# tingiskhan/pyfilter

Hardware: AMD Instinct MI355X
Metric: particle-steps/sec (batch x particles x T), 1M-particle APF (higher is better)
Workload: dtype f32; 1 GPU; apf_lgo_1m: APF + lgo proposal, systematic resampling, N=1048576 particles x B=1 filters per GPU, T=250, state dim 1; parallelism=single GPU

## Files before the change

### pyfilter_amd/csrc/pf_fused.hpp

```cpp
#pragma once

namespace pf {

#define PF_STEP_B blockIdx.x
#define PF_STEP_K blockIdx.y

#ifdef PF_DEVTOOLS
#define PF_CUT(a, n) ((a).debug_cut == (n))
#define PF_STAMP(a, slot)                                                                       \
    do {                                                                                        \
        if ((a).debug_cut < 0 && !(a).finalize_only && PF_STEP_K == (unsigned)(-(a).debug_cut - 1) &&  \
            PF_STEP_B == 0 && threadIdx.x == 0)                                                 \
            (a).dbg[slot] = (unsigned long long)clock64();                                      \
    } while (0)
#else
#define PF_CUT(a, n) false
#ifdef PF_ISA_MARKS
#define PF_STAMP(a, slot) asm volatile("; PF_MARK " #slot)
#else
#define PF_STAMP(a, slot) do { } while (0)
#endif
#endif

template <typename T> struct FusedArgs {
    ModelDesc md;
    const T* params;
    int filter, proposal, resampler;
    Geom g;
    double thr_abs;
    double logN;
    T rcN;
    uint64_t seed;
    const uint64_t* seed_dev;
    T* x[2];
    T* logw[2];
    int32_t* anc;
    const int32_t* anc_prev;
    T* cdf;
    T* pos;
    const T* y;
    int y_rows;
    const T* z_tape;
    const T* u_tape;
    const T* user_loc;
    const T* user_scale;
    int user_scale_percol;
    T user_dt;
    T* means;
    T* vars;
    T* ll_steps;
    T* ll_total;
    double* part;
    int64_t part_stride;
    ColStat* stat;
    int32_t* poison;
    T* cpack;
    double* piv0;
    double* ctab;
    int64_t ctab_stride;
    int t0;
    int step;
    int obs;
    int obs_next;
    const uint8_t* obs_dev;
    __device__ __forceinline__ bool y_informative() const {
        const T* yr = y + (int64_t)step * md.obs_dim;
        bool any = false;
        for (int o = 0; o < md.obs_dim; ++o) any = any || !(yr[o] != yr[o]);
        return any;
    }
    __device__ __forceinline__ bool is_obs() const { return obs >= 0 ? obs != 0 : (obs == -1 ? obs_dev[step] != 0 : y_informative()); }
    __device__ __forceinline__ bool is_obs_next() const { return obs_next >= 0 ? obs_next != 0 : obs_dev[step + 1] != 0; }
    int finalize_only;
    int book_inline;
    unsigned kmap;
    __device__ __forceinline__ int tile_of_row(unsigned y) const {
        return (int)(((y & (kmap & 0xffu)) << ((kmap >> 8) & 0xffu)) + (y >> ((kmap >> 16) & 0xffu)));
    }
    unsigned long long* dbg;
    __device__ __forceinline__ const double* part_r() const { return part + (int64_t)(step & 1) * part_stride; }
    __device__ __forceinline__ double* part_w(int state) const { return part + (int64_t)(state & 1) * part_stride; }
    __device__ __forceinline__ const double* ctab_r(int b) const {
        return ctab + (int64_t)(step & 1) * ctab_stride + (int64_t)b * g.tiles * g.rounds_per_tile * PF_NWAVES * 2;
    }
    __device__ __forceinline__ double* ctab_w(int state, int b) const {
        return ctab + (int64_t)(state & 1) * ctab_stride + (int64_t)b * g.tiles * g.rounds_per_tile * PF_NWAVES * 2;
    }
    template <int D> __device__ __forceinline__ T pivot(int q, int b, int d) const {
        return (q - 2 >= t0) ? means[((int64_t)(q - 2) * g.B + b) * D + d] : (T)piv0[(int64_t)b * PF_MAXD + d];
    }
    int debug_cut;
};

template <typename T, int D>
__device__ __forceinline__ void load_col_params(const FusedArgs<T>& a, int b, int step, bool with_y, ColParams<T, D>& cp,
                                                int late = 0) {
    const int O = a.md.obs_dim;
    const int NP = 4 * D + O * D + 2 * O;
    cp.load(a.params + (int64_t)b * NP + late, O,
            with_y ? a.y + ((int64_t)step * a.y_rows + (a.y_rows == 1 ? 0 : b)) * O + late : nullptr);
}

template <typename T, int D, bool WQ = true> struct PartialAcc {
    T m1, m2;
    T s1, s2, q1;
    T mx[D], mxx[D];
    double es;
    bool poison;
    __device__ __forceinline__ void init() {
        m1 = m2 = -Lim<T>::inf();
        s1 = s2 = q1 = T(0);
        es = 0.0;
#pragma unroll
        for (int d = 0; d < D; ++d) mx[d] = mxx[d] = T(0);
        poison = false;
    }
    template <int VEC>
    __device__ __forceinline__ void push_round(const T (&lw)[VEC], const T (&x)[D][VEC], bool pre_on, const T (&pre)[VEC],
                                               const T (&piv)[D], T (&e_out)[VEC]) {
        T m = lw[0];
#pragma unroll
        for (int j = 1; j < VEC; ++j) m = (lw[j] > m) ? lw[j] : m;
        if (m > m1) {
            const T rs = (m1 == -Lim<T>::inf()) ? T(0) : pf_exp_w(m1 - m);
            s1 *= rs;
            if constexpr (WQ) q1 *= rs * rs;
#pragma unroll
            for (int d = 0; d < D; ++d) {
                mx[d] *= rs;
                mxx[d] *= rs;
            }
            m1 = m;
        }
#pragma unroll
        for (int j = 0; j < VEC; ++j) {
            T e = (lw[j] == -Lim<T>::inf()) ? T(0) : pf_exp_w(lw[j] - m1);
            if (lw[j] != lw[j]) e = lw[j];
            e_out[j] = e;
            s1 += e;
            if constexpr (WQ) q1 += e * e;
#pragma unroll
            for (int d = 0; d < D; ++d) {
                const T xd = x[d][j] - piv[d];
                mx[d] += e * xd;
                mxx[d] += e * xd * xd;
            }
        }
        if (pre_on) {
            T rw[VEC];
#pragma unroll
            for (int j = 0; j < VEC; ++j) {
                if (is_nan_or_posinf(pre[j])) poison = true;
                rw[j] = sanitize_logw(pre[j] + lw[j]);
            }
            T mm = rw[0];
#pragma unroll
            for (int j = 1; j < VEC; ++j) mm = (rw[j] > mm) ? rw[j] : mm;
            if (mm > m2) {
                s2 *= (m2 == -Lim<T>::inf()) ? T(0) : pf_exp_w(m2 - mm);
                m2 = mm;
            }
#pragma unroll
            for (int j = 0; j < VEC; ++j) {
                const T e = (rw[j] == -Lim<T>::inf()) ? T(0) : pf_exp_w(rw[j] - m2);
                e_out[j] = e;
                s2 += e;
            }
        }
    }
    template <bool WITH_ES>
    __device__ __forceinline__ void finish(double* part, int b, int k, int B, int tiles, bool pre_on, double* red, T* redm,
                                           int32_t* poison_slot, T& M1_out, T& M2_out, T& F1_out, T& F2_out) {
        const int lane = threadIdx.x & 63, wid = threadIdx.x >> 6;
        const T w1 = wave_max<T>(m1), w2 = wave_max<T>(m2);
        if (lane == 0) {
            redm[wid] = w1;
            redm[PF_NWAVES + wid] = w2;
        }
        __syncthreads();
        T M1 = redm[0], M2 = redm[PF_NWAVES];
#pragma unroll
        for (int w = 1; w < PF_NWAVES; ++w) {
            M1 = (redm[w] > M1) ? redm[w] : M1;
            M2 = (redm[PF_NWAVES + w] > M2) ? redm[PF_NWAVES + w] : M2;
        }
        M1_out = M1;
        M2_out = M2;
        const T f1 = (m1 == -Lim<T>::inf()) ? T(0) : pf_exp_w(m1 - M1);
        const T f2 = (!pre_on || m2 == -Lim<T>::inf()) ? T(0) : pf_exp_w(m2 - M2);
        F1_out = f1;
        F2_out = f2;
        constexpr int NS = 3 + 2 * D;
        T sums[NS];
        sums[0] = s1 * f1;
        sums[1] = WQ ? q1 * f1 * f1 : T(0);
        sums[2] = pre_on ? s2 * f2 : T(0);
#pragma unroll
        for (int d = 0; d < D; ++d) {
            sums[3 + d] = mx[d] * f1;
            sums[3 + D + d] = mxx[d] * f1;
        }
#pragma unroll
        for (int q = 0; q < NS; ++q) {
            const T ws = (WQ || q != 1) ? wave_sum(sums[q]) : T(0);
            if (lane == 0) red[q * PF_NWAVES + wid] = (double)ws;
        }
        if constexpr (WITH_ES) {
            const double ws = wave_sum(es);
            if (lane == 0) red[NS * PF_NWAVES + wid] = ws;
        }
        if (poison) atomicOr(poison_slot, 1);
        __syncthreads();
        if (threadIdx.x < NS + 1) {
            const int q = threadIdx.x;
            double r = 0.0;
            if (q < NS || WITH_ES) {
                r = red[q * PF_NWAVES];
#pragma unroll
                for (int w = 1; w < PF_NWAVES; ++w) r += red[q * PF_NWAVES + w];
            }
            const int row = q == 0 ? PQ_S1 : q == 1 ? PQ_Q1 : q == 2 ? PQ_S2 : q == NS ? PQ_E : PQ_MX + (q - 3);
            const int64_t stride = (int64_t)B * tiles;
            const int64_t o = (int64_t)b * tiles + k;
            part[row * stride + o] = r;
            if (q == 0) {
                part[PQ_M1 * stride + o] = (double)M1;
                part[PQ_M2 * stride + o] = pre_on ? (double)M2 : -__builtin_huge_val();
            }
        }
    }
};

#define PF_LDS_CHUNKS PF_WAVE
template <typename T>
__device__ __forceinline__ T cdf_from_local(T L, double Pk, double fk, double Pnext, bool tile_last, bool col_last) {
    double c = Pk + fk * (double)L;
    if (c > Pnext) c = Pnext;
    T r = (T)c;
    if (tile_last) r = col_last ? T(1) : (T)Pnext;
    return r;
}
template <typename T>
__device__ __forceinline__ T cdf_from_local(T L, double C, double gq, double Pk, double fk, double Pnext, bool tile_last,
                                            bool col_last) {
    double c = Pk + fk * (C + gq * (double)L);
    if (c > Pnext) c = Pnext;
    T r = (T)c;
    if (tile_last) r = col_last ? T(1) : (T)Pnext;
    return r;
}
template <typename T> struct CdfView {
    const T* L;
    const double* ptab;
    const double* ftab;
    const double* ct;
    int chunk_elems;
    int N;
    int tile_elems;
    int tiles;
    __device__ __forceinline__ int lower_bound(int from, T p, int kt_lo) const {
        if (from >= N) return N;
        int lo = kt_lo, hi = tiles - 1;
        while (lo < hi) {
            const int mid = (lo + hi) >> 1;
            if ((T)ptab[mid + 1] < p) lo = mid + 1; else hi = mid;
        }
        for (int kt = lo; kt < tiles; ++kt) {
            const int first = kt * tile_elems;
            const int end = first + tile_elems < N ? first + tile_elems : N;
            int a = from > first ? from : first, b = end;
            if (a >= b) continue;
            const double Pk = ptab[kt], fk = ftab[kt], Pn = ptab[kt + 1];
            while (a < b) {
                const int mid = (a + b) >> 1;
                T cv;
                if (ct) {
                    const double* cg = ct + 2 * (mid / chunk_elems);
                    cv = cdf_from_local<T>(L[mid], cg[0], cg[1], Pk, fk, Pn, mid == end - 1, mid == N - 1);
                } else {
                    cv = cdf_from_local<T>(L[mid], Pk, fk, Pn, mid == end - 1, mid == N - 1);
                }
                if (cv < p) a = mid + 1; else b = mid;
            }
            if (a < end) return a;
        }
        return N;
    }
};

template <typename T, int VEC, bool WT = false>
__device__ __forceinline__ void chunk_scan_round(const T (&rw)[VEC], bool on, T* __restrict__ l_base, int l_elem, int chunk,
                                                 double* lds_rec, double* raw) {
    T* const l_dst = l_base + l_elem;
    const int lane = threadIdx.x & 63;
    T mt = rw[0];
// ... 71 lines not shown
    const Geom& g = a.g;
    const int b = blockIdx.y, k = blockIdx.x;
    const int slot = a.step & 1;
    const bool pre_on = a.is_obs() && a.filter == PF_FILTER_APF;
    const bool user = a.md.hid_kind == PF_HID_USER_AFFINE;
    ColParams<T, D> cp;
    load_col_params<T, D>(a, b, a.step, pre_on, cp);
    ColConsts<T, D> cc;
    cc.prepare(a.md, cp);
    if (user && a.user_scale_percol) cc.prepare_user(a.md, cp, a.user_scale[b]);

    const T* lw_col = a.logw[slot] + (int64_t)b * g.N;
    const T* x_base = a.x[slot];
    T piv[D];
#pragma unroll
    for (int d = 0; d < D; ++d) piv[d] = x_base[((int64_t)d * g.B + b) * g.N];
    if (k == 0 && threadIdx.x == 0) {
#pragma unroll
        for (int d = 0; d < D; ++d) a.piv0[(int64_t)b * PF_MAXD + d] = (double)piv[d];
    }
    if constexpr (D == 1) {
        if (k == 0 && threadIdx.x == PF_BLOCK - 1 && a.md.obs_kind == PF_OBS_LINEAR && a.md.hid_kind != PF_HID_VERHULST_EM) {
            ColParams<T, 1> cq;
            ColConsts<T, 1> cd;
            load_col_params<T, 1>(a, b, a.step, false, cq);
            cd.prepare(a.md, cq);
            write_col_pack<T>(a.md, cq, cd, a.cpack + (int64_t)b * PK_N);
        }
    }
    PartialAcc<T, D> acc;
    acc.init();
    __shared__ double reds[PF_NWAVES];
    __shared__ double crec[2 * PF_LDS_CHUNKS];
    const bool use_lds = g.rounds_per_tile * PF_NWAVES <= PF_LDS_CHUNKS;
    double* const ct_tile = a.ctab_w(a.step, b) + 2 * (int64_t)k * g.rounds_per_tile * PF_NWAVES;
    T* const l_col = ((a.step & 1) ? a.pos : a.cdf) + (int64_t)b * g.N;
    const int64_t base = (int64_t)k * g.tile_elems;
    int rk = 0;
    for (int r = 0; r < g.rounds_per_tile; ++r) {
        const int64_t r0 = base + (int64_t)r * g.round_elems;
        if (r0 >= g.N) break;
        ++rk;
        const int64_t i0 = r0 + threadIdx.x * VEC;
        const bool on = i0 < g.N;
        T rw[VEC];
#pragma unroll
        for (int j = 0; j < VEC; ++j) rw[j] = -Lim<T>::inf();
        if (on) {
            T lw[VEC], xv[D][VEC];
            if (VEC == 1) lw[0] = lw_col[i0]; else load_vec<T, VEC>(lw_col + i0, lw);
#pragma unroll
            for (int d = 0; d < D; ++d) {
                const T* xc = x_base + ((int64_t)d * g.B + b) * g.N + i0;
                if (VEC == 1) xv[d][0] = xc[0]; else load_vec<T, VEC>(xc, xv[d]);
            }
            T pre[VEC];
#pragma unroll
            for (int j = 0; j < VEC; ++j) {
                T xj[D];
#pragma unroll
                for (int d = 0; d < D; ++d) xj[d] = xv[d][j];
                UserMS<T, D> um = UserMS<T, D>::none();
                if (user && pre_on) {
                    um.gather(a.user_loc, a.user_scale, (int64_t)b * g.N, (int64_t)g.B * g.N, i0 + j, a.user_scale_percol != 0, b, g.B);
                    um.euler(xj, a.user_dt);
                }
                pre[j] = pre_on ? pre_weight<T, D>(a.md, a.proposal, cp, cc, xj, false, um) : T(0);
                if (pre_on && is_nan_or_posinf(pre[j])) acc.poison = true;
                rw[j] = pre_on ? sanitize_logw(pre[j] + lw[j]) : lw[j];
            }
            T e_unused[VEC];
            acc.template push_round<VEC>(lw, xv, false, pre, piv, e_unused);
            if (a.resampler == PF_RESAMPLE_MULTINOMIAL) {
                T ev[VEC];
                draw_exponentials<T, VEC>(a.seed + (a.seed_dev ? *a.seed_dev : 0ull), PF_STREAM_MULTINOMIAL, (uint32_t)a.step,
                                          (uint64_t)((int64_t)b * g.N + i0), ev);
#pragma unroll
                for (int j = 0; j < VEC; ++j) acc.es += (double)ev[j];
            }
        }
        chunk_scan_round<T, VEC>(rw, on, l_col + r0, threadIdx.x * VEC, r * PF_NWAVES + (threadIdx.x >> 6), use_lds ? crec : nullptr, ct_tile);
    }
    T M1, M2, F1, F2;
    acc.template finish<true>(a.part_w(a.step), b, k, g.B, g.tiles, false, red, redm, &a.poison[(a.step & 3) * g.B + b], M1, M2, F1, F2);
    double Mc, Sc;
    finalize_chunk_table<T>(ct_tile, use_lds ? crec : nullptr, rk * PF_NWAVES, reds, redm, Mc, Sc);
    if (threadIdx.x == 0) {
        const int64_t stride = (int64_t)g.B * g.tiles, o = (int64_t)b * g.tiles + k;
        if (pre_on) {
            a.part_w(a.step)[PQ_M2 * stride + o] = Mc;
            a.part_w(a.step)[PQ_S2 * stride + o] = Sc;
        } else {
            a.part_w(a.step)[PQ_S1 * stride + o] = Sc;
        }
    }
    if (g.rounds_per_tile == 1) {
        __syncthreads();
        const int64_t i0 = base + threadIdx.x * VEC;
        if (i0 < g.N) {
            const double* cg = ct_tile + 2 * (threadIdx.x >> 6);
            const double C = cg[0], gq = cg[1];
            T v[VEC];
            if (VEC == 1) v[0] = l_col[i0]; else load_vec<T, VEC>(l_col + i0, v);
#pragma unroll
            for (int j = 0; j < VEC; ++j) v[j] = (T)(C + gq * (double)v[j]);
            if (VEC == 1) l_col[i0] = v[0]; else store_vec<T, VEC>(l_col + i0, v);
        }
    }
}

#define PF_COMBINE_ITERS (PF_MAX_TILES / PF_BLOCK)
template <typename T> __device__ __forceinline__ double pf_rcp_tot(double tot) {
    if constexpr (sizeof(T) == 4) {
        double r = __builtin_amdgcn_rcp(tot);
        r = __builtin_fma(__builtin_fma(-tot, r, 1.0), r, r);
        r = __builtin_fma(__builtin_fma(-tot, r, 1.0), r, r);
        return r;
    }
    return 1.0 / tot;
}
#define PF_PROBE_STEP 8
struct ColSums {
    double M, S, Q;
};
template <bool WITH_Q, int NX> struct ColPartials {
    double m[PF_COMBINE_ITERS], s[PF_COMBINE_ITERS], q[PF_COMBINE_ITERS];
    double x[NX ? NX : 1][PF_COMBINE_ITERS];
};
template <bool WITH_Q, int NX = 0>
__device__ __forceinline__ void load_col_partials(const double* part, int64_t stride, int64_t cb, int tiles, int slot_m,
                                                  int slot_s, int slot_x, ColPartials<WITH_Q, NX>& r) {
    const int IT = (tiles + PF_BLOCK - 1) / PF_BLOCK;
    if constexpr (PF_COMBINE_ITERS == 4 && NX == 0) {
        if (IT == 4 && (tiles & 3) == 0) {
            const int t0 = threadIdx.x * 4;
            if (t0 < tiles) {
                double a2[2], b2[2];
                const double* pm = part + slot_m * stride + cb + t0;
                load_vec<double, 2>(pm, a2); load_vec<double, 2>(pm + 2, b2);
                r.m[0] = a2[0]; r.m[1] = a2[1]; r.m[2] = b2[0]; r.m[3] = b2[1];
                const double* ps = part + slot_s * stride + cb + t0;
                load_vec<double, 2>(ps, a2); load_vec<double, 2>(ps + 2, b2);
                r.s[0] = a2[0]; r.s[1] = a2[1]; r.s[2] = b2[0]; r.s[3] = b2[1];
                if constexpr (WITH_Q) {
                    const double* pq = part + PQ_Q1 * stride + cb + t0;
                    load_vec<double, 2>(pq, a2); load_vec<double, 2>(pq + 2, b2);
                    r.q[0] = a2[0]; r.q[1] = a2[1]; r.q[2] = b2[0]; r.q[3] = b2[1];
                } else {
                    r.q[0] = r.q[1] = r.q[2] = r.q[3] = 0.0;
                }
            } else {
#pragma unroll
                for (int q = 0; q < 4; ++q) { r.m[q] = -__builtin_huge_val(); r.s[q] = 0.0; r.q[q] = 0.0; }
            }
            return;
        }
    }
#pragma unroll
    for (int q = 0; q < PF_COMBINE_ITERS; ++q) {
        const int t = threadIdx.x * IT + q;
        const bool on = q < IT && t < tiles;
        r.m[q] = on ? part[slot_m * stride + cb + t] : -__builtin_huge_val();
        r.s[q] = on ? part[slot_s * stride + cb + t] : 0.0;
        r.q[q] = (WITH_Q && on) ? part[PQ_Q1 * stride + cb + t] : 0.0;
#pragma unroll
        for (int i = 0; i < NX; ++i) r.x[i][q] = on ? part[(slot_x + i) * stride + cb + t] : 0.0;
    }
// ... 598 lines not shown
                    const double Ca = cga[0], ga = cga[1], Cb = cgb[0], gb = cgb[1];
#pragma unroll
                    for (int j = 0; j < VEC; ++j) {
                        const bool tl = (j == VEC - 1) && (wja + j == la);
                        m0[j] = wina ? cdf_from_local<T>(m0[j], Ca, ga, tPa, tFa, tNa, tl, tl && (wja + j == N - 1)) : Lim<T>::inf();
                    }
#pragma unroll
                    for (int j = 0; j < V1; ++j)
                        m1[j] = winb ? cdf_from_local<T>(m1[j], Cb, gb, tPb, tFb, tNb, wjb + j == lb, wjb + j == N - 1) : Lim<T>::inf();
                } else {
#pragma unroll
                    for (int j = 0; j < VEC; ++j) {
                        const bool tl = (j == VEC - 1) && (wja + j == la);
                        m0[j] = wina ? cdf_from_local<T>(m0[j], tPa, tFa, tNa, tl, tl && (wja + j == N - 1)) : Lim<T>::inf();
                    }
#pragma unroll
                    for (int j = 0; j < V1; ++j)
                        m1[j] = winb ? cdf_from_local<T>(m1[j], tPb, tFb, tNb, wjb + j == lb, wjb + j == N - 1) : Lim<T>::inf();
                }
            };
            map_window(ws, ja, jb, ina, inb, c0, c1);
            if (XWIN) {
#pragma unroll
                for (int d = 0; d < D; ++d) {
                    if (ina) { if (VEC == 1) xwin[d * WIN + tid] = xa[d][0]; else store_vec<T, VEC>(xwin + d * WIN + tid * VEC, xa[d]); }
                    if (inb) { if (V1 == 1) xwin[d * WIN + PF_BLOCK * VEC + tid] = xb[d][0]; else store_vec<T, V1>(xwin + d * WIN + PF_BLOCK * VEC + tid * V1, xb[d]); }
                }
            }
            if constexpr (MODE != 0) {
                if (VEC == 1) { win[tid] = c0[0]; win[PF_BLOCK + tid] = c1[0]; }
                else { store_vec<T, VEC>(win + tid * VEC, c0); store_vec<T, VEC>(win + (PF_BLOCK + tid) * VEC, c1); }
                __syncthreads();
                T pp[VEC];
                int qq[VEC];
#pragma unroll
                for (int j = 0; j < VEC; ++j) pp[j] = multinomial ? pv[j] : grid_position<T>(i0 + j, ub, nT);
                window_lower_bound_flat<T, WIN, VEC>(win, pp, qq);
#pragma unroll
                for (int j = 0; j < VEC; ++j) {
                    const int64_t i = i0 + j;
                    int res = N - 1;
                    if (i < N) {
                        res = (qq[j] < WIN) ? ws + qq[j] : view.lower_bound(ws + WIN < N ? ws + WIN : N, pp[j], kt0);
                        if (res > N - 1) res = N - 1;
                    }
                    idx[j] = res;
                }
            } else {
                inverse_grid_round<T, VEC, V1>(c0, c1, ws, (int)r0, g.round_elems, N, ub, nT, rcN, pow2, i0, hd, sh_cl, sh_wm,
                                           [&](int it, T (&d0)[VEC], T (&d1)[V1]) -> bool {
                                               const int w0 = ws + it * STAGED;
                                               if (w0 >= N) return false;
                                               const int wja = w0 + tid * VEC, wjb = w0 + PF_BLOCK * VEC + tid * V1;
                                               const bool wina = wja < N, winb = wjb < N;
                                               if (wina) { if (VEC == 1) d0[0] = cdf_col[wja]; else load_vec<T, VEC>(cdf_col + wja, d0); }
                                               if (winb) { if (V1 == 1) d1[0] = cdf_col[wjb]; else load_vec<T, V1>(cdf_col + wjb, d1); }
                                               map_window(w0, wja, wjb, wina, winb, d0, d1);
                                               return true;
                                           },
                                           [&](int64_t i, int from) { return view.lower_bound(from, grid_position<T>(i, ub, nT), from ? kt0 : 0); },
                                           idx);
            }
            if (r + 1 < g.rounds_per_tile) {
                if (tid == PF_BLOCK - 1) sh_j0 = idx[VEC - 1];
                __syncthreads();
                j0 = sh_j0;
            }
        } else {
#pragma unroll
            for (int j = 0; j < VEC; ++j) idx[j] = (int)((i0 + j < g.N) ? (i0 + j) : (g.N - 1));
        }
        PF_STAMP(a, 11);
#ifdef PF_DEVTOOLS
        if (on && PF_CUT(a, 2)) {
            if (VEC == 1) anc_col[i0] = idx[0]; else store_vec<int, VEC>(anc_col + i0, idx);
        }
#endif

        int late;
        asm volatile("v_readfirstlane_b32 %0, %1\n\ts_and_b32 %0, %0, 0" : "=s"(late) : "v"(idx[0]) : "scc");
        using KArgs = const __attribute__((address_space(4))) FusedArgs<T>;
        KArgs* la = (KArgs*)((const_ptr<char>)__builtin_amdgcn_kernarg_segment_ptr() + late);
        T* const x_out = la->x[slot ^ 1];
#ifndef PF_DEVTOOLS
        T* const lw_out = la->logw[slot ^ 1] + (int64_t)b * g.N;
        int32_t* const anc_col = la->anc + (int64_t)b * g.N;
#endif
        if constexpr (FAST) {
            const_ptr<T> yq = (const_ptr<T>)(uintptr_t)a.y + late;
            const int yc = a.y_rows == 1 ? 0 : b;
            const T y_t = obs ? yq[(int64_t)step * a.y_rows + yc] : T(0);
            const T y_n = pre_next ? yq[(int64_t)(step + 1) * a.y_rows + yc] : T(0);
            fc.load((const_ptr<T>)(uintptr_t)(a.cpack + (int64_t)b * PK_N) + late, y_t, y_n);
        } else if constexpr (D == 1) {
            load_col_params<T, D>(a, b, step, obs, cp, late);
            if (pre_next) cp.load_next(a.y + ((int64_t)(step + 1) * a.y_rows + (a.y_rows == 1 ? 0 : b)) * a.md.obs_dim + late);
            cc.prepare(md, cp);
            if constexpr (USER) {
                if (la->user_scale_percol) cc.prepare_user(md, cp, la->user_scale[b]);
            } else {
                __builtin_assume(cc.fast == FAST);
            }
        } else if (r == 0) {
            cc.prepare(md, cp);
            __builtin_assume(cc.fast == FAST);
        }
        T xo[D][VEC];
        if (on && !PF_CUT(a, 2)) {
            T lwo[VEC], pre_n[VEC];
            T xr[VEC][D];
            if (!resample) {
#pragma unroll
                for (int d = 0; d < D; ++d) {
                    T xv[VEC];
                    const T* xc = x_in + ((int64_t)d * g.B + b) * g.N + i0;
                    if (VEC == 1) xv[0] = xc[0]; else load_vec<T, VEC>(xc, xv);
#pragma unroll
                    for (int j = 0; j < VEC; ++j) xr[j][d] = xv[j];
                }
            } else {
#pragma unroll
                for (int j = 0; j < VEC; ++j) {
                    const int q = idx[j] - ws;
                    const bool in_lds = XWIN && windowed && q >= 0 && q < STAGED;
#pragma unroll
                    for (int d = 0; d < D; ++d)
                        xr[j][d] = in_lds ? xwin[d * WIN + q] : x_in[((int64_t)d * g.B + b) * g.N + idx[j]];
                }
            }
#pragma unroll
            for (int j = 0; j < VEC; ++j) {
                T xn[D];
                T w_new;
                UserMS<T, D> um = UserMS<T, D>::none();
                if constexpr (USER) {
                    um.gather(la->user_loc, la->user_scale, (int64_t)b * g.N, (int64_t)g.B * g.N, idx[j], la->user_scale_percol != 0, b, g.B);
                    um.euler(xr[j], la->user_dt);
                }
                if (obs) {
                    T wi, pre_anc = T(0);
                    if constexpr (FAST) {
                        if (apf) wi = fc.template sample_and_weight_apf<FAST ? MK : 0>(proposal, xr[j][0], zt[j][0], xn[0], pre_anc);
                        else wi = fc.template sample_and_weight<FAST ? MK : 0>(proposal, xr[j][0], zt[j][0], xn[0]);
                    } else {
                        wi = sample_and_weight<T, D>(md, proposal, cp, cc, xr[j], zt[j], xn, um);
                    }
                    if (apf) {
                        if constexpr (FAST) w_new = wi - pre_anc;
                        else w_new = wi - pre_weight<T, D>(md, proposal, cp, cc, xr[j], false, um);
                        if (is_nan_or_posinf(w_new)) poison = true;
                    } else {
                        if (is_nan_or_posinf(wi)) poison = true;
                        w_new = resample ? wi : (wi + lw_old[j]);
                    }
                } else {
                    if constexpr (FAST) fc.template sample_and_weight<FAST ? MK : 0>(PF_PROP_BOOTSTRAP, xr[j][0], zt[j][0], xn[0]);
                    else sample_and_weight<T, D>(md, PF_PROP_BOOTSTRAP, cp, cc, xr[j], zt[j], xn, um);
                    w_new = resample ? T(0) : lw_old[j];
                }
                lwo[j] = sanitize_logw(w_new);
#pragma unroll
                for (int d = 0; d < D; ++d) xo[d][j] = xn[d];
                if constexpr (FAST) pre_n[j] = pre_next ? fc.template pre_weight<FAST ? MK : 0>(proposal, xn[0], true) : T(0);
                else if constexpr (USER) {
                    pre_n[j] = pre_next ? pre_weight<T, D>(md, proposal, cp, cc, xn, true, um) : T(0);
                } else pre_n[j] = pre_next ? pre_weight<T, D>(md, proposal, cp, cc, xn, true) : T(0);
                if (j & 1) __builtin_amdgcn_sched_barrier(0);
            }
            PF_STAMP(a, 12);
#pragma unroll
            for (int d = 0; d < D; ++d) {
                T* xc = x_out + ((int64_t)d * g.B + b) * g.N + r0;
                if (VEC == 1) xc[tid] = xo[d][0]; else store_out<T, VEC, !MULTI>(xc, tid * VEC, xo[d]);
            }
            if (VEC == 1) lw_out[i0] = lwo[0]; else store_out<T, VEC, !MULTI>(lw_out + r0, tid * VEC, lwo);
            if (resample || apf) {
                if (VEC == 1) anc_col[i0] = idx[0]; else store_out<int, VEC, !MULTI>(anc_col + r0, tid * VEC, idx);
            } else if (la->anc_prev) {
                const int32_t* ap = la->anc_prev + (int64_t)b * g.N + i0;
                int prev[VEC];
                if (VEC == 1) prev[0] = ap[0]; else load_vec<int, VEC>(ap, prev);
                if (VEC == 1) anc_col[i0] = prev[0]; else store_vec<int, VEC>(anc_col + i0, prev);
            }
            if (PF_CUT(a, 5)) {
                if (pre_next) { if (VEC == 1) lw_out[i0] = pre_n[0]; else store_vec<T, VEC>(lw_out + i0, pre_n); }
                continue;
            }
            T piv[D];
#pragma unroll
            for (int d = 0; d < D; ++d)
                piv[d] = (step - 1 >= a.t0) ? la->means[((int64_t)(step - 1) * g.B + b) * D + d] : (T)la->piv0[(int64_t)b * PF_MAXD + d];
            if constexpr (MULTI) {
#pragma unroll
                for (int j = 0; j < VEC; ++j) {
                    if (pre_next && is_nan_or_posinf(pre_n[j])) acc.poison = true;
                    rwn[j] = pre_next ? sanitize_logw(pre_n[j] + lwo[j]) : lwo[j];
                }
            }
            acc.template push_round<VEC>(lwo, xo, single && pre_next, pre_n, piv, e_rw);
            if (multinomial) {
                T ev[VEC];
                draw_exponentials<T, VEC>(seed, PF_STREAM_MULTINOMIAL, (uint32_t)(step + 1), (uint64_t)((int64_t)b * g.N + i0), ev);
#pragma unroll
                for (int j = 0; j < VEC; ++j) acc.es += (double)ev[j];
            }
            PF_STAMP(a, 13);
        }
        if (scan_next && !single) {
            chunk_scan_round<T, VEC, false>(rwn, on, l_next + r0, tid * VEC, r * PF_NWAVES + (tid >> 6), use_lds ? sh.crec : nullptr, ct_tile);
#pragma unroll
            for (int j = 0; j < VEC; ++j) rwn[j] = -Lim<T>::inf();
            ++rk;
        }
        if (windowed && r + 1 < g.rounds_per_tile) __syncthreads();
    }
    if (poison) atomicOr(&a.poison[(step & 3) * g.B + b], 1);
    if (PF_CUT(a, 3)) return;
    PF_STAMP(a, 14);
    T M1, M2, F1, F2;
    acc.template finish<MODE == 1>(a.part_w(step + 1), b, k, g.B, g.tiles, single && pre_next, red, redm, &a.poison[((step + 1) & 3) * g.B + b], M1, M2, F1, F2);
    if (PF_CUT(a, 6)) return;
    if (scan_next && single) {
        const int64_t i0 = base + tid * VEC;
        const bool on = i0 < g.N;
        const T f = pre_next ? F2 : F1;
        double e[VEC], local = 0.0, total;
#pragma unroll
        for (int j = 0; j < VEC; ++j) {
            local += on ? (double)(e_rw[j] * f) : 0.0;
            e[j] = local;
        }
        const double excl = block_scan_excl(local, reds, total);
        if (on) {
            T outv[VEC];
#pragma unroll
            for (int j = 0; j < VEC; ++j) outv[j] = (T)(excl + e[j]);
            if (VEC == 1) l_next[i0] = outv[0]; else store_out<T, VEC, !MULTI>(l_next + base, tid * VEC, outv);
        }
    } else if (scan_next) {
        double Mc, Sc;
        finalize_chunk_table<T>(ct_tile, use_lds ? sh.crec : nullptr, rk * PF_NWAVES, reds, redm, Mc, Sc);
        if (tid == 0) {
            const int64_t stride = (int64_t)g.B * g.tiles, o = (int64_t)b * g.tiles + k;
            if (pre_next) {
                a.part_w(step + 1)[PQ_M2 * stride + o] = Mc;
                a.part_w(step + 1)[PQ_S2 * stride + o] = Sc;
            } else {
                a.part_w(step + 1)[PQ_S1 * stride + o] = Sc;
            }
        }
    }
    PF_STAMP(a, 15);
#ifdef PF_DEVTOOLS
    if (a.debug_cut < 0 && tid == 0 && b == 0 && (k % 128) == 0 && k / 128 < 8) a.dbg[24 + k / 128] = wall_clock64();
#endif
}

template <typename T, int D, int VEC, int MODE, int PROP, bool FAST, int SPEC, int MK, bool MULTI>
__global__ __launch_bounds__(PF_BLOCK, (StepWaves<T, D, MODE, PROP, FAST, SPEC, MULTI>::value)) void k_fused_step(FusedArgs<T> a) {
    using SH = StepShared<T, D, VEC>;
    __shared__ __attribute__((aligned(32))) T win[SH::WIN];
    __shared__ __attribute__((aligned(32))) T xwin[SH::XWIN ? D * SH::WIN : VEC];
    __shared__ int sh_j0;
    __shared__ int sh_cl[2 * PF_NWAVES], sh_wm[PF_NWAVES];
    __shared__ double red[(4 + 2 * D) * PF_NWAVES];
    __shared__ double reds[PF_NWAVES];
    __shared__ T redm[2 * PF_NWAVES];
    __shared__ double ptl[PF_MAX_TILES + 2], ftl[PF_MAX_TILES];
    __shared__ int sh_plan[2];
    __shared__ double crec[MULTI ? 2 * PF_LDS_CHUNKS : 2];
    __shared__ double redb[PF_NWAVES];
    if (!a.book_inline && PF_STEP_K == (unsigned)a.g.tiles) {
        column_bookkeeping<T, D>(a, PF_STEP_B, red, redb);
        return;
    }
    const SH sh{win, xwin, &sh_j0, sh_cl, sh_wm, red, reds, redm, ptl, ftl, sh_plan, crec};
    T z0[VEC][D];
#pragma unroll
    for (int j = 0; j < VEC; ++j)
#pragma unroll
        for (int d = 0; d < D; ++d) z0[j][d] = T(0);
    const StepPlan<T> pl = step_prologue<T, D, VEC, MODE, SPEC, (FAST && D == 1 && sizeof(T) == 4), MULTI>(a, sh, z0);
    if constexpr (SPEC == 1) {
        step_body<T, D, VEC, MODE, PROP, FAST, SPEC, MK, true, MULTI>(a, sh, pl, z0);
    } else {
        if (pl.resample) step_body<T, D, VEC, MODE, PROP, FAST, SPEC, MK, true, MULTI>(a, sh, pl, z0);
        else step_body<T, D, VEC, MODE, PROP, FAST, SPEC, MK, false, MULTI>(a, sh, pl, z0);
    }
    if (a.book_inline == 1 && PF_STEP_K == (unsigned)a.g.tiles - 1u)
        column_bookkeeping<T, D>(a, PF_STEP_B, red, redb);
}

template <typename W> __global__ __launch_bounds__(PF_BLOCK) void k_zero_words(W* __restrict__ p, size_t n) {
    const size_t i = (size_t)blockIdx.x * PF_BLOCK + threadIdx.x;
    if (i < n) p[i] = W(0);
}

template <typename T>
__global__ __launch_bounds__(PF_WAVE) void k_observed_flags(const T* __restrict__ y, int64_t row_elems, uint8_t* __restrict__ out) {
    const T* row = y + (int64_t)blockIdx.x * row_elems;
    bool any = false;
    for (int64_t i = threadIdx.x; i < row_elems; i += PF_WAVE) any |= !(row[i] != row[i]);
    const unsigned long long bal = __ballot(any);
    if (threadIdx.x == 0) out[blockIdx.x] = bal ? 1 : 0;
}

template <typename T>
__global__ __launch_bounds__(PF_BLOCK) void k_zero_and_flags(uint32_t* __restrict__ p, size_t n, unsigned zero_blocks, const T* __restrict__ y,
                                                             int64_t row_elems, uint8_t* __restrict__ out) {
    if (blockIdx.x < zero_blocks) {
        const size_t i = (size_t)blockIdx.x * PF_BLOCK + threadIdx.x;
        if (i < n) p[i] = 0u;
        return;
    }
    if (threadIdx.x >= PF_WAVE) return;
    const unsigned k = blockIdx.x - zero_blocks;
    const T* row = y + (int64_t)k * row_elems;
    bool any = false;
    for (int64_t i = threadIdx.x; i < row_elems; i += PF_WAVE) any |= !(row[i] != row[i]);
    const unsigned long long bal = __ballot(any);
    if (threadIdx.x == 0) out[k] = bal ? 1 : 0;
}
// ... 36 lines not shown
```

### pyfilter_amd/csrc/pf_kernels.hip

```cpp
#include <hip/hip_runtime.h>
#include <stdint.h>

#include <atomic>
#include <cstdlib>
#include <cstring>
#include <mutex>
#include <vector>

#include <type_traits>

#include "../../include/pf_amd.h"
#include "pf_device.hpp"
#include "pf_models.hpp"
#include "pf_philox.hpp"
#include "pf_linear.hpp"

namespace pf {

#define PF_MAX_TILES 1024
#define PF_TARGET_WGS 1024
#define PF_AUTO_FLAGS 128

struct Geom {
    int64_t N;
// ... 2104 lines not shown
            });
        });
    });
}

#endif

#define PF_TRACE_LEN 2048
#define PF_TRACE_FIELDS 10
struct LaunchTrace {
    int32_t rec[PF_TRACE_LEN][PF_TRACE_FIELDS];
    uint64_t count;
};
LaunchTrace& launch_trace();
static inline void trace_launch(int step, int tbytes, int d, int vec, int mode, int prop, int fast, int spec, int mk, int multi) {
    LaunchTrace& t = launch_trace();
    int32_t* r = t.rec[t.count % PF_TRACE_LEN];
    r[0] = step; r[1] = tbytes; r[2] = d; r[3] = vec; r[4] = mode; r[5] = prop; r[6] = fast; r[7] = spec; r[8] = mk; r[9] = multi;
    ++t.count;
}
#ifndef PF_TU_NO_API
LaunchTrace& launch_trace() {
    static thread_local LaunchTrace t = {};
    return t;
}
extern "C" int pf_debug_launch_trace(int32_t* out, int max_records) {
    if (!out || max_records < 0) return PF_EINVAL;
    const LaunchTrace& t = launch_trace();
    const uint64_t have = t.count < PF_TRACE_LEN ? t.count : PF_TRACE_LEN;
    const int n = (uint64_t)max_records < have ? max_records : (int)have;
    for (int i = 0; i < n; ++i)
        for (int f = 0; f < PF_TRACE_FIELDS; ++f) out[i * PF_TRACE_FIELDS + f] = t.rec[(t.count - n + i) % PF_TRACE_LEN][f];
    return n;
}
#endif

template <typename T>
static FusedArgs<T> make_fused_args(const pf_filter_args* A, const Geom& g, const WsLayout& wl, int64_t t0) {
    FusedArgs<T> a;
    a.md = to_desc(&A->model);
    a.params = (const T*)A->model.params;
    a.filter = A->filter;
    a.proposal = A->proposal;
    a.resampler = A->resampler;
    a.g = g;
    a.thr_abs = A->ess_threshold * (double)A->N;
    a.logN = log((double)A->N);
    a.rcN = T(1) / T(A->N);
    a.seed = A->seed;
    a.seed_dev = (const uint64_t*)A->step_counter;
    a.x[0] = (T*)A->x[0];
    a.x[1] = (T*)A->x[1];
    a.logw[0] = (T*)A->logw[0];
    a.logw[1] = (T*)A->logw[1];
    a.anc = A->anc;
    a.anc_prev = nullptr;
    a.cdf = (T*)A->cdf;
    a.pos = (T*)A->pos;
    a.y = (const T*)A->y;
    a.y_rows = (int)A->y_rows;
    a.z_tape = (const T*)A->z_tape;
    a.u_tape = (const T*)A->u_tape;
    a.user_loc = (const T*)A->user_loc;
    a.user_scale = (const T*)A->user_scale;
    a.user_scale_percol = A->user_scale_per_column != 0 ? 1 : 0;
    a.user_dt = (T)A->user_dt;
    a.means = (T*)A->means;
    a.vars = (T*)A->vars;
    a.ll_steps = (T*)A->ll_steps;
    a.ll_total = (T*)A->ll_total;
    a.part = (double*)((char*)A->ws + wl.off_part);
    a.part_stride = (int64_t)wl.part_elems;
    a.stat = (ColStat*)((char*)A->ws + wl.off_stat);
    a.poison = (int32_t*)((char*)A->ws + wl.off_poison);
    a.dbg = (unsigned long long*)((char*)A->ws + wl.off_dbg);
    a.cpack = (T*)((char*)A->ws + wl.off_cpack);
    a.piv0 = (double*)((char*)A->ws + wl.off_piv0);
    a.ctab = (double*)((char*)A->ws + wl.off_ctab);
    a.ctab_stride = (int64_t)wl.ctab_elems;
    static_assert(PK_N == 24, "workspace layout reserves 24 slots per column record");
    a.finalize_only = 0;
    a.t0 = (int)t0;
    a.debug_cut = 0;
#ifdef PF_DEVTOOLS
    if (const char* dc = getenv("PF_DEBUG_CUT")) a.debug_cut = atoi(dc);
#endif
    return a;
}

template <typename T>
struct ObsFlags {
    const uint8_t* host;
    const uint8_t* dev;
    bool inline_y;
    bool derive;
    uint8_t* slot;
    int64_t row;
    const T* y;

    ObsFlags(const pf_filter_args* A, const WsLayout& wl, int64_t t0, int64_t n_steps) {
        const bool none = !A->observed && !A->observed_dev && n_steps > 0;
        host = A->observed;
        inline_y = none && n_steps == 1 && A->y_rows == 1;
        derive = none && !inline_y;
        slot = (uint8_t*)A->ws + wl.off_ctr + 64;
        row = A->y_rows * (int64_t)A->model.obs_dim;
        y = derive ? (const T*)A->y + t0 * row : nullptr;
        dev = derive ? slot - t0 : A->observed_dev;
    }
    int obs(int64_t t) const { return inline_y ? -2 : dev ? -1 : (host[t] != 0); }
    void launch_derive(int64_t n_steps, hipStream_t st) const {
        hipLaunchKernelGGL((k_observed_flags<T>), dim3((unsigned)n_steps), dim3(PF_WAVE), 0, st, y, row, slot);
    }
    void launch_zero(uint32_t* p, size_t words, bool flags, int64_t n_steps, hipStream_t st) const {
        const unsigned zb = (unsigned)((words + PF_BLOCK - 1) / PF_BLOCK);
        if (flags)
            hipLaunchKernelGGL((k_zero_and_flags<T>), dim3(zb + (unsigned)n_steps), dim3(PF_BLOCK), 0, st, p, words, zb, y, row, slot);
        else
            hipLaunchKernelGGL((k_zero_words<uint32_t>), dim3(zb), dim3(PF_BLOCK), 0, st, p, words);
    }
    ColumnRun piece(int64_t t, int64_t left) const {
        ColumnRun r;
        r.t0 = (int)t;
        r.n_steps = (int)(left < 32 * PFC_OBS_WORDS ? left : 32 * PFC_OBS_WORDS);
        r.use_bits = (dev == nullptr && !inline_y) ? 1 : 0;
        r.inline_y = inline_y ? 1 : 0;
        for (int w = 0; w < PFC_OBS_WORDS; ++w) r.obs_bits[w] = 0u;
        if (r.use_bits)
            for (int q = 0; q < r.n_steps; ++q)
                if (host[r.t0 + q]) r.obs_bits[q >> 5] |= 1u << (q & 31);
        return r;
    }
};

struct KernelTimer {
    float* kernel_ms;
    hipStream_t st;
    hipEvent_t ev[2] = {nullptr, nullptr};
    bool failed = false;
    int rc = PF_OK;
    KernelTimer(float* kernel_ms_, hipStream_t st_) : kernel_ms(kernel_ms_), st(st_) {
        if (!kernel_ms) return;
        for (auto& e : ev)
            if (hipEventCreate(&e) != hipSuccess) {
                failed = true;
                rc = (int)hipGetLastError();
                return;
            }
        (void)hipEventRecord(ev[0], st);
    }
    ~KernelTimer() {
        for (auto& e : ev)
            if (e) (void)hipEventDestroy(e);
    }
    void stop() const {
        if (kernel_ms) (void)hipEventRecord(ev[1], st);
    }
    int finish(int64_t n_steps) const {
        if (!kernel_ms) return PF_OK;
        const hipError_t se = hipStreamSynchronize(st);
        if (se != hipSuccess) return (int)se;
        float ms = 0.f;
        (void)hipEventElapsedTime(&ms, ev[0], ev[1]);
        kernel_ms[0] = kernel_ms[2] = n_steps > 0 ? ms / (float)n_steps : 0.f;
        kernel_ms[1] = 0.f;
        return PF_OK;
// ... 64 lines not shown
    a.obs_dev = flags.dev;
    if (flags.derive && t0 != 0) flags.launch_derive(n_steps, st);
    a.obs = n_steps > 0 ? flags.obs(t0) : 0;
    a.obs_next = 0;
    const bool resumed = A->hints.resume != 0 && t0 > 0 && A->ring < 3;
    const bool prepare_next = A->hints.prepare_next != 0 && A->filter == PF_FILTER_APF && !finalize && n_steps > 0;
    if (!resumed) hipLaunchKernelGGL((k_fused_reduce<T, D, VEC>), grid_tiles, block, 0, st, a);

    const bool force_search = A->hints.ancestor_search != 0;
    const int mode = (A->resampler == PF_RESAMPLE_MULTINOMIAL)
                         ? 1
                         : ((sizeof(T) == 4 && (g.N > ((int64_t)1 << 22) || force_search)) ? 2 : 0);
    auto spec_of = [&]() -> int {
        if (sizeof(T) != 4 || a.z_tape || a.obs != 1) return 0;
        if (a.md.hid_kind == PF_HID_USER_AFFINE && a.filter == PF_FILTER_APF) return 0;
        if (a.filter == PF_FILTER_APF) return a.obs_next == 1 ? 1 : 0;
        return 2;
    };
    auto launch_step_as = [&](auto prop_c, auto fast_c) {
        constexpr int PROP = decltype(prop_c)::value;
        constexpr bool FAST = decltype(fast_c)::value;
        auto go = [&](auto mode_c, auto spec_c) {
            constexpr int MODE = decltype(mode_c)::value;
            constexpr int SPEC = decltype(spec_c)::value;
            auto launch = [&](auto mk_c) {
                constexpr int MK = decltype(mk_c)::value;
                trace_launch((int)a.step, (int)sizeof(T), D, VEC, MODE, PROP, FAST ? 1 : 0, SPEC, MK, MULTI ? 1 : 0);
                hipLaunchKernelGGL((k_fused_step<T, D, VEC, MODE, PROP, FAST, SPEC, MK, MULTI>), grid, block, 0, st, a);
            };
            if constexpr (!FAST) {
                if (a.md.hid_kind == PF_HID_USER_AFFINE) {
                    if constexpr (SPEC != 1) launch(std::integral_constant<int, 3>{});
                    return;
                }
            }
            if constexpr (sizeof(T) == 4 && !FAST && D == 1) {
                if (a.md.hid_kind == PF_HID_VERHULST_EM && a.md.obs_kind == PF_OBS_SV) return launch(std::integral_constant<int, 1>{});
            }
            if constexpr (sizeof(T) == 4 && !FAST && D == 3) {
                if (a.md.hid_kind == PF_HID_LORENZ63_EM && a.md.obs_kind == PF_OBS_LINEAR)
                    return launch(std::integral_constant<int, 4>{});
            }
            if constexpr (sizeof(T) == 4 && FAST && D == 1) {
                if (a.md.hid_kind == PF_HID_SINE_EM) return launch(std::integral_constant<int, 2>{});
                return launch(std::integral_constant<int, 1>{});
            }
            launch(std::integral_constant<int, 0>{});
        };
        auto with_mode = [&](auto mode_c) {
            if constexpr (sizeof(T) == 4) {
                const int sp = spec_of();
                if (sp == 1) return go(mode_c, std::integral_constant<int, 1>{});
                if (sp == 2) return go(mode_c, std::integral_constant<int, 2>{});
            }
            go(mode_c, std::integral_constant<int, 0>{});
        };
        if (mode == 0) with_mode(std::integral_constant<int, 0>{});
        else if (mode == 1) with_mode(std::integral_constant<int, 1>{});
        else if constexpr (sizeof(T) == 4) go(std::integral_constant<int, 2>{}, std::integral_constant<int, 0>{});
    };
    auto launch_step = [&]() {
        bool fast = false;
        if constexpr (D == 1)
            fast = a.md.obs_kind == PF_OBS_LINEAR && a.md.hid_kind != PF_HID_VERHULST_EM && a.md.hid_kind != PF_HID_USER_AFFINE;
        if (fast) {
            if constexpr (D == 1) {
                if (a.proposal == PF_PROP_BOOTSTRAP) launch_step_as(std::integral_constant<int, PF_PROP_BOOTSTRAP>{}, std::true_type{});
                else launch_step_as(std::integral_constant<int, PF_PROP_LGO>{}, std::true_type{});
            }
        } else if (a.proposal == PF_PROP_BOOTSTRAP) {
            launch_step_as(std::integral_constant<int, PF_PROP_BOOTSTRAP>{}, std::false_type{});
        } else {
            launch_step_as(std::integral_constant<int, PF_PROP_LGO>{}, std::false_type{});
        }
    };
    const KernelTimer timer(kernel_ms, st);
    if (timer.failed) return timer.rc;
    for (int64_t s = 0; s < n_steps; ++s) {
        const int64_t t = t0 + s;
        a.step = (int)t;
        place(t);
        a.obs = flags.obs(t);
        a.obs_next = (s + 1 < n_steps) ? flags.obs(t + 1) : (prepare_next ? 1 : 0);
#ifdef PF_DEVTOOLS
        static const bool cut_at_end = getenv("PF_DEBUG_CUT_AT_END") != nullptr;
        const int cut_all = a.debug_cut;
        if (cut_at_end && cut_all > 0 && s != n_steps - 2) a.debug_cut = 0;
#endif
        launch_step();
#ifdef PF_DEVTOOLS
        a.debug_cut = cut_all;
#endif
    }
    timer.stop();
    if (finalize) {
        a.step = (int)(t0 + n_steps);
        a.obs = a.obs_next = 0;
        a.finalize_only = 1;
        hipLaunchKernelGGL((k_fused_book<T, D>), dim3(1, g.B), block, 0, st, a);
    }
    if (const int rc = timer.finish(n_steps)) return rc;
    return launch_status();
}

#define PF_LEAF_AT(T, D, VEC, MULTI) \
    template int filter_run_impl<T, D, VEC, MULTI>(const pf_filter_args*, const Geom&, const WsLayout&, int64_t, int64_t, int, hipStream_t, float*);
#ifdef PF_TU_MULTI
#define PF_LEAF(T, D, VEC) PF_LEAF_AT(T, D, VEC, PF_TU_MULTI != 0)
#else
#define PF_LEAF(T, D, VEC) PF_LEAF_AT(T, D, VEC, false) PF_LEAF_AT(T, D, VEC, true)
#endif
#if !defined(PF_TU_NO_F32D1) && !defined(PF_TU_F64_ONLY) && !defined(PF_TU_F32DN_ONLY)
#if !defined(PF_TU_VEC) || PF_TU_VEC == 4
PF_LEAF(float, 1, 4)
#endif
#if !defined(PF_TU_VEC) || PF_TU_VEC == 1
PF_LEAF(float, 1, 1)
#endif
#endif
#if !defined(PF_TU_NO_F32DN) && !defined(PF_TU_F64_ONLY) && !defined(PF_TU_F32D1_ONLY)
PF_LEAF(float, 2, 4) PF_LEAF(float, 3, 4) PF_LEAF(float, 2, 1) PF_LEAF(float, 3, 1)
#endif
#if !defined(PF_TU_NO_F64) && !defined(PF_TU_F32DN_ONLY) && !defined(PF_TU_F32D1_ONLY)
PF_LEAF(double, 1, 4) PF_LEAF(double, 2, 4) PF_LEAF(double, 3, 4) PF_LEAF(double, 1, 1) PF_LEAF(double, 2, 1) PF_LEAF(double, 3, 1)
#endif
#undef PF_LEAF
#undef PF_LEAF_AT
#endif

static inline int column_threads(int64_t N, int vec) {
    const int64_t need = (N + vec - 1) / vec;
    return (int)(((need + PF_WAVE - 1) / PF_WAVE) * PF_WAVE);
}
#define PF_COLUMN_VEC 4
static inline size_t column_lds_bytes(int64_t N, int D, size_t tsize, int vec) {
    int64_t np2 = 64;
    while (np2 < N) np2 <<= 1;
    const int64_t NP = ((N + vec - 1) / vec) * vec;
    const size_t planes = (((size_t)(np2 + PF_LB_PAD + (int64_t)D * NP) * tsize) + 15) & ~(size_t)15;
    return planes + sizeof(double) * (2 + 2 * (4 + 2 * D)) * PFC_MAXW + 16;
}
#define PF_COLUMN_MAX_N 2048
static inline bool column_eligible(const pf_filter_args* A, const Geom& g, int64_t n_steps, int finalize) {
    if (!finalize || n_steps < 1 || A->ring >= 3) return false;
    if (A->hints.route == PF_ROUTE_PER_STEP) return false;
    const int64_t max_n = A->hints.column_max_n > 0 ? A->hints.column_max_n : PF_COLUMN_MAX_N;
    if (A->N > max_n || column_threads(A->N, PF_COLUMN_VEC) > 1024) return false;
    return column_lds_bytes(A->N, A->model.dim, A->dtype == PF_F64 ? 8 : 4, PF_COLUMN_VEC) <= 64 * 1024;
}

template <typename T, int D>
static int column_run_impl(const pf_filter_args* A, const Geom& g, const WsLayout& wl, int64_t t0, int64_t n_steps,
                           hipStream_t st, float* kernel_ms) {
    constexpr int VEC = PF_COLUMN_VEC;
    FusedArgs<T> a = make_fused_args<T>(A, g, wl, t0);
    const int nt = column_threads(A->N, VEC);
    const size_t lds = column_lds_bytes(A->N, D, sizeof(T), VEC);
    const ObsFlags<T> flags(A, wl, t0, n_steps);
    a.obs_dev = flags.dev;
    if (flags.derive) flags.launch_derive(n_steps, st);
    const KernelTimer timer(kernel_ms, st);
    if (timer.failed) return timer.rc;
    auto with_column_folded = [&](auto&& f) {
        if (A->hints.route == PF_ROUTE_COLUMN_GENERIC) return false;
        if constexpr (sizeof(T) == 4 && D == 1) return with_folded<PF_HID_LINEAR, PF_HID_SINE_EM, PF_HID_OU, PF_HID_VERHULST_EM>(A, f);
        if constexpr (sizeof(T) == 4 && D == 3) return A->N % VEC == 0 && with_folded<PF_HID_LORENZ63_EM>(A, f);
        return false;
// ... 313 lines not shown
```

Before: 76.36 billion particle-steps/s.

## Skip dead ancestor/logw stores in APF steps and fuse tile scan into finish barrier

Adds a keep_state flag that is set only on the last step or when a ring buffer is active. On intermediate APF steps this lets the kernel skip writing ancestor indices and log-weights that the next step would not read. For the single-tile VEC=4 path it also folds the next-step prefix scan into the reduction barrier in finish(), removing a separate block_scan and its extra syncs. The cost is more complex correctness conditions around when state must be kept, plus extra live registers across the barrier.

```diff
diff --git a/pyfilter_amd/csrc/pf_fused.hpp b/pyfilter_amd/csrc/pf_fused.hpp
--- a/pyfilter_amd/csrc/pf_fused.hpp
+++ b/pyfilter_amd/csrc/pf_fused.hpp
@@ -90,6 +90,7 @@
         return (q - 2 >= t0) ? means[((int64_t)(q - 2) * g.B + b) * D + d] : (T)piv0[(int64_t)b * PF_MAXD + d];
     }
     int debug_cut;
+    int keep_state;
 };
 
 template <typename T, int D>
@@ -168,9 +169,9 @@
             }
         }
     }
-    template <bool WITH_ES>
+    template <bool WITH_ES, typename FB, typename FA>
     __device__ __forceinline__ void finish(double* part, int b, int k, int B, int tiles, bool pre_on, double* red, T* redm,
-                                           int32_t* poison_slot, T& M1_out, T& M2_out, T& F1_out, T& F2_out) {
+                                           int32_t* poison_slot, T& M1_out, T& M2_out, T& F1_out, T& F2_out, FB&& before, FA&& after) {
         const int lane = threadIdx.x & 63, wid = threadIdx.x >> 6;
         const T w1 = wave_max<T>(m1), w2 = wave_max<T>(m2);
         if (lane == 0) {
@@ -210,7 +211,9 @@
             if (lane == 0) red[NS * PF_NWAVES + wid] = ws;
         }
         if (poison) atomicOr(poison_slot, 1);
+        before(f1, f2);
         __syncthreads();
+        after();
         if (threadIdx.x < NS + 1) {
             const int q = threadIdx.x;
             double r = 0.0;
@@ -448,7 +451,7 @@
         chunk_scan_round<T, VEC>(rw, on, l_col + r0, threadIdx.x * VEC, r * PF_NWAVES + (threadIdx.x >> 6), use_lds ? crec : nullptr, ct_tile);
     }
     T M1, M2, F1, F2;
-    acc.template finish<true>(a.part_w(a.step), b, k, g.B, g.tiles, false, red, redm, &a.poison[(a.step & 3) * g.B + b], M1, M2, F1, F2);
+    acc.template finish<true>(a.part_w(a.step), b, k, g.B, g.tiles, false, red, redm, &a.poison[(a.step & 3) * g.B + b], M1, M2, F1, F2, [](T, T) {}, []() {});
     double Mc, Sc;
     finalize_chunk_table<T>(ct_tile, use_lds ? crec : nullptr, rk * PF_NWAVES, reds, redm, Mc, Sc);
     if (threadIdx.x == 0) {
@@ -1213,10 +1216,6 @@
         using KArgs = const __attribute__((address_space(4))) FusedArgs<T>;
         KArgs* la = (KArgs*)((const_ptr<char>)__builtin_amdgcn_kernarg_segment_ptr() + late);
         T* const x_out = la->x[slot ^ 1];
-#ifndef PF_DEVTOOLS
-        T* const lw_out = la->logw[slot ^ 1] + (int64_t)b * g.N;
-        int32_t* const anc_col = la->anc + (int64_t)b * g.N;
-#endif
         if constexpr (FAST) {
             const_ptr<T> yq = (const_ptr<T>)(uintptr_t)a.y + late;
             const int yc = a.y_rows == 1 ? 0 : b;
@@ -1299,24 +1298,36 @@
                 if (j & 1) __builtin_amdgcn_sched_barrier(0);
             }
             PF_STAMP(a, 12);
+            const bool keep = la->keep_state != 0;
+            const bool st_anc = keep || !apf;
+            const bool st_lw = keep || !(apf && obs && pre_next);
 #pragma unroll
             for (int d = 0; d < D; ++d) {
                 T* xc = x_out + ((int64_t)d * g.B + b) * g.N + r0;
                 if (VEC == 1) xc[tid] = xo[d][0]; else store_out<T, VEC, !MULTI>(xc, tid * VEC, xo[d]);
             }
-            if (VEC == 1) lw_out[i0] = lwo[0]; else store_out<T, VEC, !MULTI>(lw_out + r0, tid * VEC, lwo);
+            if (st_lw) {
+                T* const lw_st = la->logw[slot ^ 1] + (int64_t)b * g.N;
+                if (VEC == 1) lw_st[i0] = lwo[0]; else store_out<T, VEC, !MULTI>(lw_st + r0, tid * VEC, lwo);
+            }
             if (resample || apf) {
-                if (VEC == 1) anc_col[i0] = idx[0]; else store_out<int, VEC, !MULTI>(anc_col + r0, tid * VEC, idx);
+                if (st_anc) {
+                    int32_t* const anc_st = la->anc + (int64_t)b * g.N;
+                    if (VEC == 1) anc_st[i0] = idx[0]; else store_out<int, VEC, !MULTI>(anc_st + r0, tid * VEC, idx);
+                }
             } else if (la->anc_prev) {
                 const int32_t* ap = la->anc_prev + (int64_t)b * g.N + i0;
+                int32_t* const anc_st = la->anc + (int64_t)b * g.N;
                 int prev[VEC];
                 if (VEC == 1) prev[0] = ap[0]; else load_vec<int, VEC>(ap, prev);
-                if (VEC == 1) anc_col[i0] = prev[0]; else store_vec<int, VEC>(anc_col + i0, prev);
-            }
+                if (VEC == 1) anc_st[i0] = prev[0]; else store_vec<int, VEC>(anc_st + i0, prev);
+            }
+#ifdef PF_DEVTOOLS
             if (PF_CUT(a, 5)) {
                 if (pre_next) { if (VEC == 1) lw_out[i0] = pre_n[0]; else store_vec<T, VEC>(lw_out + i0, pre_n); }
                 continue;
             }
+#endif
             T piv[D];
 #pragma unroll
             for (int d = 0; d < D; ++d)
@@ -1349,26 +1360,56 @@
     if (PF_CUT(a, 3)) return;
     PF_STAMP(a, 14);
     T M1, M2, F1, F2;
-    acc.template finish<MODE == 1>(a.part_w(step + 1), b, k, g.B, g.tiles, single && pre_next, red, redm, &a.poison[((step + 1) & 3) * g.B + b], M1, M2, F1, F2);
+    constexpr bool fused_tail = single && MODE != 1 && VEC == 4;
+    const bool tile_scan = scan_next && fused_tail;
+    const int64_t i0s = base + tid * VEC;
+    const bool on_s = i0s < g.N;
+    double e[VEC], local = 0.0, incl = 0.0;
+    acc.template finish<MODE == 1>(a.part_w(step + 1), b, k, g.B, g.tiles, single && pre_next, red, redm, &a.poison[((step + 1) & 3) * g.B + b], M1, M2, F1, F2,
+        [&](T f1, T f2) {
+            if (!tile_scan) return;
+            const T f = pre_next ? f2 : f1;
+#pragma unroll
+            for (int j = 0; j < VEC; ++j) {
+                local += on_s ? (double)(e_rw[j] * f) : 0.0;
+                e[j] = local;
+            }
+            incl = wave_scan_incl(local, tid & 63);
+            if ((tid & 63) == 63) reds[tid >> 6] = incl;
+        },
+        [&]() {
+            if (!tile_scan) return;
+            double wave_off = 0.0;
+#pragma unroll
+            for (int w = 0; w < PF_NWAVES; ++w) {
+                const double sw = reds[w];
+                if (w < (tid >> 6)) wave_off += sw;
+            }
+            const double excl = wave_off + incl - local;
+            if (on_s) {
+                T outv[VEC];
+#pragma unroll
+                for (int j = 0; j < VEC; ++j) outv[j] = (T)(excl + e[j]);
+                if (VEC == 1) l_next[i0s] = outv[0]; else store_out<T, VEC, !MULTI>(l_next + base, tid * VEC, outv);
+            }
+        });
     if (PF_CUT(a, 6)) return;
-    if (scan_next && single) {
-        const int64_t i0 = base + tid * VEC;
-        const bool on = i0 < g.N;
+    if (scan_next && single && !fused_tail) {
         const T f = pre_next ? F2 : F1;
-        double e[VEC], local = 0.0, total;
+        double total;
 #pragma unroll
         for (int j = 0; j < VEC; ++j) {
-            local += on ? (double)(e_rw[j] * f) : 0.0;
+            local += on_s ? (double)(e_rw[j] * f) : 0.0;
             e[j] = local;
         }
         const double excl = block_scan_excl(local, reds, total);
-        if (on) {
+        if (on_s) {
             T outv[VEC];
 #pragma unroll
             for (int j = 0; j < VEC; ++j) outv[j] = (T)(excl + e[j]);
-            if (VEC == 1) l_next[i0] = outv[0]; else store_out<T, VEC, !MULTI>(l_next + base, tid * VEC, outv);
-        }
-    } else if (scan_next) {
+            if (VEC == 1) l_next[i0s] = outv[0]; else store_out<T, VEC, !MULTI>(l_next + base, tid * VEC, outv);
+        }
+    } else if (scan_next && !single) {
         double Mc, Sc;
         finalize_chunk_table<T>(ct_tile, use_lds ? sh.crec : nullptr, rk * PF_NWAVES, reds, redm, Mc, Sc);
         if (tid == 0) {
diff --git a/pyfilter_amd/csrc/pf_kernels.hip b/pyfilter_amd/csrc/pf_kernels.hip
--- a/pyfilter_amd/csrc/pf_kernels.hip
+++ b/pyfilter_amd/csrc/pf_kernels.hip
@@ -2210,6 +2210,7 @@
     a.finalize_only = 0;
     a.t0 = (int)t0;
     a.debug_cut = 0;
+    a.keep_state = 1;
 #ifdef PF_DEVTOOLS
     if (const char* dc = getenv("PF_DEBUG_CUT")) a.debug_cut = atoi(dc);
 #endif
@@ -2440,7 +2441,9 @@
         place(t);
         a.obs = flags.obs(t);
         a.obs_next = (s + 1 < n_steps) ? flags.obs(t + 1) : (prepare_next ? 1 : 0);
+        a.keep_state = (ring != 0 || s + 1 == n_steps) ? 1 : 0;
 #ifdef PF_DEVTOOLS
+        if (a.debug_cut != 0) a.keep_state = 1;
         static const bool cut_at_end = getenv("PF_DEBUG_CUT_AT_END") != nullptr;
         const int cut_all = a.debug_cut;
         if (cut_at_end && cut_all > 0 && s != n_steps - 2) a.debug_cut = 0;
```

Result: faster. 78.50 billion particle-steps/s, median of 6 (+2.8%).
